# Agzs/BlockMaze

Measured on AMD Instinct MI355X. Metric: Groth16 proofs/sec (send circuit, alt_bn128), higher is better.
Workload: dtype u32 limbs (254-bit Fq/Fr Montgomery; all MSM accumulations, the H query's weighted bucket sum and the transforms' tiles on nine 29-bit limbs)

## Files before the change

### blockmaze_amd/csrc/capi_engine.cpp

```cpp
#include <cstring>
#include <memory>
#include <mutex>
#include <string>
#include <vector>
#include "../../include/zkgpu.h"
#include "gpu.hpp"
#include "capi_accounts.hpp"

namespace zk {
void probe_field(int field, int op, const uint8_t *a, const uint8_t *b, uint8_t *out, size_t n);
void probe_fq2(int op, const uint8_t *a, const uint8_t *b, uint8_t *out, size_t n);
void probe_group(int group, int op, const uint8_t *a, const uint8_t *b, uint8_t *out, size_t n);
void probe_field29(int field, int op, const uint32_t *a, const uint32_t *b, const uint32_t *c, const uint32_t *d, uint32_t *out, size_t n);
void probe_point29(int op, const uint32_t *a, const uint32_t *b, uint32_t *out, uint32_t *flags, size_t n);
void probe_fq2_sqrt(const uint8_t *a, uint8_t *out, uint8_t *ok, size_t n);
}
using namespace zk;
using namespace zk::host;

static thread_local std::string g_err;
void zkgpu_set_error(const std::string &s) { g_err = s; }
std::mutex g_gpu_mutex;

template <class Fn> static int guarded(Fn fn) {
// ... 153 lines not shown
void zkgpu_r1cs_destroy(zkgpu_r1cs *cs) { guarded([&] { delete cs; return ZKGPU_OK; }); }
int zkgpu_witness_map(zkgpu_r1cs *cs, const uint8_t *z, uint8_t *h_out) { return guarded([&] { if (!cs) return ZKGPU_ERR_ARG;
  size_t m = cs->dom->m(), nv = cs->host.n_vars; std::vector<Fe32> zz(nv + 1); memset(&zz[0], 0, 32); zz[0].l[0] = 1; if (nv) memcpy(&zz[1], z, 32 * nv);
  DevBuf<Fe32> zd(nv + 1), abc(3 * m); zd.upload(zz.data(), nv + 1); fr_to_mont_dev(zd.get(), nv + 1);
  cs->dev->eval(zd.get(), abc.get(), m);
  if (!cs->dev->satisfied(abc.get(), m)) {
    g_err = "assignment does not satisfy the constraint system";
    return ZKGPU_ERR_UNSATISFIED;
  }
  cs->dom->ifft(abc.get(), 3, m);
  cs->dom->coset_fft(abc.get(), 3, m);
  cs->dom->qap_pointwise(abc.get(), abc.get() + m, abc.get() + 2 * m);
  cs->dom->icoset_fft(abc.get(), 1, m);
  fr_from_mont_dev(abc.get(), m); abc.download((Fe32 *)h_out, m); memset(h_out + 32 * m, 0, 32); return ZKGPU_OK; }); }

int zkgpu_test_decompress(int group, const uint8_t *xs_mont, const uint8_t *flags, size_t n, uint8_t *points_out) {
  return guarded([&] { if (group != 1 && group != 2) { g_err = "group must be 1 or 2"; return ZKGPU_ERR_ARG; }
    if (group == 1) { std::vector<G1AffineRaw> p(n ? n : 1); decompress_g1((const Fe32 *)xs_mont, flags, n, p.data()); for (size_t i = 0; i < n; i++) g1_raw_out(p[i], points_out + 64 * i); }
    else { std::vector<G2AffineRaw> p(n ? n : 1); decompress_g2((const Fe32 *)xs_mont, flags, n, p.data()); for (size_t i = 0; i < n; i++) g2_raw_out(p[i], points_out + 128 * i); }
    return ZKGPU_OK; });
}
int zkgpu_test_fixed_base_mul(int group, const uint8_t *base, const uint8_t *scalars, size_t n, uint8_t *points_out) {
  return guarded([&] { if (group != 1 && group != 2) { g_err = "group must be 1 or 2"; return ZKGPU_ERR_ARG; }
    if (group == 1) { G1AffineRaw b; g1_to_raw(base, b); HFq x, y; memcpy(x.l, &b.x, 32); memcpy(y.l, &b.y, 32);
      std::vector<G1AffineRaw> p(n ? n : 1); fixed_base_mul_g1(HG1::from_affine(x, y), (const Fe32 *)scalars, n, p.data()); for (size_t i = 0; i < n; i++) g1_raw_out(p[i], points_out + 64 * i); }
    else { G2AffineRaw b; g2_to_raw(base, b); HFq2 x, y; memcpy(x.c0.l, &b.x0, 32); memcpy(x.c1.l, &b.x1, 32); memcpy(y.c0.l, &b.y0, 32); memcpy(y.c1.l, &b.y1, 32);
      std::vector<G2AffineRaw> p(n ? n : 1); fixed_base_mul_g2(HG2::from_affine(x, y), (const Fe32 *)scalars, n, p.data()); for (size_t i = 0; i < n; i++) g2_raw_out(p[i], points_out + 128 * i); }
    return ZKGPU_OK; });
}
int zkgpu_test_h_query_lagrange(size_t min_size, const uint8_t *h, size_t n_in, uint8_t *out) {
// ... 72 lines not shown
```

### blockmaze_amd/csrc/gpu.hip

```cpp
#include <hip/hip_runtime.h>
#include <cstdio>
#include <cstdlib>
#include <chrono>
#include <cstring>
#include <map>
#include <vector>
#include <algorithm>
#include <mutex>
#include <atomic>
#include <mutex>
#include "gpu_internal.hpp"
#include "ntt.cuh"
#include "ecntt.cuh"

__attribute__((constructor(101))) static void zkgpu_load_time_environment() { setenv("GPU_MAX_HW_QUEUES", "16", 0); }

namespace zk {

constexpr int MAX_LANES_PER_DEVICE = 31, MAX_LANES = 1 + 8 * 28;
static uint8_t g_lane_claimed[MAX_LANES];
static std::atomic<GpuContext *> g_lanes[MAX_LANES];
static std::atomic<int> g_lane_slot[MAX_LANES];
static std::mutex g_lane_mutex;
static thread_local int t_lane = 0;
// ... 198 lines not shown
    o.n_ = 0;
  }
  return *this;
}
template <class T> void DevBuf<T>::upload(const T *h, size_t n) {
  HIP_CHECK(hipMemcpyAsync(p_, h, n * sizeof(T), hipMemcpyHostToDevice, gpu().stream));
  HIP_CHECK(hipStreamSynchronize(gpu().stream));
}
template <class T> void DevBuf<T>::download(T *h, size_t n) const {
  HIP_CHECK(hipMemcpyAsync(h, p_, n * sizeof(T), hipMemcpyDeviceToHost, gpu().stream));
  HIP_CHECK(hipStreamSynchronize(gpu().stream));
}
template <class T> void DevBuf<T>::zero() { if (n_) HIP_CHECK(hipMemsetAsync(p_, 0, n_ * sizeof(T), gpu().stream)); }
template class DevBuf<uint8_t>;
template class DevBuf<uint32_t>;
template class DevBuf<Fe32>;
template class DevBuf<G1AffineRaw>;
template class DevBuf<G2AffineRaw>;

template <class T> PinnedBuf<T>::PinnedBuf(size_t n) : n_(n) { gpu(); if (n) { HIP_CHECK(hipHostMalloc((void **)&p_, n * sizeof(T))); if (alloc_poison()) memset(p_, 0xA5, n * sizeof(T)); } }
template <class T> PinnedBuf<T>::~PinnedBuf() { release(); }
template <class T> void PinnedBuf<T>::release() { if (p_) hipHostFree(p_); p_ = nullptr; n_ = 0; }
template class PinnedBuf<Fe32>;
void upload_async(void *dev, const void *host, size_t bytes) { HIP_CHECK(hipMemcpyAsync(dev, host, bytes, hipMemcpyHostToDevice, gpu().stream)); }
static __global__ void k_copy_words16(const uint4 *__restrict__ src, uint4 *__restrict__ dst, size_t n16) {
  for (size_t i = (size_t)blockIdx.x * blockDim.x + threadIdx.x; i < n16; i += (size_t)gridDim.x * blockDim.x) dst[i] = src[i];
}
void copy_dev_async(void *dst, const void *src, size_t bytes) {
  if (!bytes) return;
  if (bytes % 16 || (reinterpret_cast<uintptr_t>(dst) | reinterpret_cast<uintptr_t>(src)) % 16) { HIP_CHECK(hipMemcpyAsync(dst, src, bytes, hipMemcpyDeviceToDevice, gpu().stream)); return; }
// ... 479 lines not shown
  return d;
}
void gpu_host_unregister(void *p) { if (p) { (void)hipHostUnregister(p); (void)hipGetLastError(); } }
static std::atomic<uint64_t> g_general_path_repeats{0}, g_queries_without_tables{0};
uint64_t queries_without_tables() { return g_queries_without_tables.load(std::memory_order_relaxed); }
void note_query_without_tables() { g_queries_without_tables.fetch_add(1, std::memory_order_relaxed); }
uint64_t general_path_repeats() { return g_general_path_repeats.load(std::memory_order_relaxed); }
void note_general_path_repeat() { g_general_path_repeats.fetch_add(1, std::memory_order_relaxed); }
void merge_equal_columns_dev(Fe32 *z, uint8_t *tags, const uint32_t *grp_ptr, const uint32_t *grp_mem, size_t n_groups) {
  if (n_groups) hipLaunchKernelGGL(k_merge_equal_columns, dim3(cdiv(n_groups, 64)), dim3(64), 0, gpu().stream, (Fr *)z, tags, grp_ptr, grp_mem, (uint32_t)n_groups);
}
void fr_to_mont_dev(Fe32 *a, size_t n) { if (n) hipLaunchKernelGGL(k_fr_to_mont, dim3(cdiv(n, 256)), dim3(256), 0, gpu().stream, (Fr *)a, (uint32_t)n); }
void fr_from_mont_dev(Fe32 *a, size_t n) { if (n) hipLaunchKernelGGL(k_fr_from_mont, dim3(cdiv(n, 256)), dim3(256), 0, gpu().stream, (Fr *)a, (uint32_t)n); }

struct R1csArrays { size_t n_inputs, n_vars, n_cons; DevBuf<uint32_t> rowptr[3], col[3], cid[3], long_rows[3]; size_t n_long[3] = {0, 0, 0}; DevBuf<Fe32> ctab;
    DevBuf<uint32_t> long_any; size_t n_long_any = 0; };
struct R1csDev::Impl {
  std::shared_ptr<R1csArrays> a;
  size_t &n_inputs, &n_vars, &n_cons;
  DevBuf<uint32_t> (&rowptr)[3], (&col)[3], (&cid)[3], (&long_rows)[3];
  size_t (&n_long)[3];
  DevBuf<Fe32> &ctab;
  DevBuf<uint32_t> &long_any;
  size_t &n_long_any;
  DevBuf<uint32_t> flag;
  uint32_t *h_flag = nullptr;
  uint32_t *h_fail = nullptr, *d_fail = nullptr, seq = 0;
  explicit Impl(std::shared_ptr<R1csArrays> aa) : a(aa), n_inputs(a->n_inputs), n_vars(a->n_vars), n_cons(a->n_cons), rowptr(a->rowptr), col(a->col),
      cid(a->cid), long_rows(a->long_rows), n_long(a->n_long), ctab(a->ctab), long_any(a->long_any), n_long_any(a->n_long_any) {
  }
  void own_words() {
    flag = DevBuf<uint32_t>(1);
    HIP_CHECK(hipHostMalloc((void **)&h_flag, 4));
    HIP_CHECK(hipHostMalloc((void **)&h_fail, 8, hipHostMallocMapped));
    h_fail[0] = 0; h_fail[1] = 0;
    HIP_CHECK(hipHostGetDevicePointer((void **)&d_fail, h_fail, 0));
  }
  ~Impl() { if (h_flag) hipHostFree(h_flag); if (h_fail) hipHostFree(h_fail); }
};
R1csDev::R1csDev(const R1csDev &peer) : impl(new Impl(peer.impl->a)) { impl->own_words(); }
R1csDev::R1csDev(const R1csHost &h) : impl(new Impl(std::make_shared<R1csArrays>())) {
  Impl &d = *impl; d.n_inputs = h.n_inputs; d.n_vars = h.n_vars; d.n_cons = h.n_cons;
  std::vector<Fe32> tab(2); { HFr one = HFr::one(), m1 = one.neg(); memcpy(&tab[0], one.l, 32); memcpy(&tab[1], m1.l, 32); }
  struct Key { uint32_t l[8]; bool operator<(const Key &o) const { return memcmp(l, o.l, 32) < 0; } };
  std::vector<std::pair<Key, uint32_t>> seen;
  size_t cap = 1 << 12; std::vector<int64_t> slots(cap, -1); std::vector<Fe32> keys; std::vector<uint32_t> vals;
  auto lookup = [&](const Fe32 &c) -> uint32_t {
    uint64_t hsh = ((uint64_t)c.l[1] << 32 | c.l[0]) * 0x9E3779B97F4A7C15ull ^ c.l[7]; size_t pos = hsh & (cap - 1);
    for (;;) { int64_t s = slots[pos]; if (s < 0) break; if (!memcmp(&keys[s], &c, 32)) return vals[s]; pos = (pos + 1) & (cap - 1); }
    if (keys.size() * 2 >= cap) throw GpuError("r1cs: more than 2048 distinct coefficients");
    HFr v; memcpy(v.l, &c, 32); v = v.to_mont(); Fe32 m; memcpy(&m, v.l, 32); uint32_t id;
    if (!memcmp(&m, &tab[0], 32)) id = 0; else if (!memcmp(&m, &tab[1], 32)) id = 1; else { id = (uint32_t)tab.size(); tab.push_back(m); }
    slots[pos] = (int64_t)keys.size(); keys.push_back(c); vals.push_back(id); return id; };
  for (int m = 0; m < 3; m++) {
    if (h.rowptr[m].size() != h.n_cons + 1) throw GpuError("r1cs: rowptr size");
    std::vector<uint32_t> ids(h.col[m].size()); for (size_t k = 0; k < ids.size(); k++) ids[k] = lookup(h.coeff[m][k]);
    d.rowptr[m] = DevBuf<uint32_t>(h.n_cons + 1); d.rowptr[m].upload(h.rowptr[m].data(), h.n_cons + 1);
    d.col[m] = DevBuf<uint32_t>(ids.size() + 1); d.cid[m] = DevBuf<uint32_t>(ids.size() + 1);
    if (!ids.empty()) { d.col[m].upload(h.col[m].data(), ids.size()); d.cid[m].upload(ids.data(), ids.size()); }
    std::vector<uint32_t> lr; for (size_t i = 0; i < h.n_cons; i++) if (h.rowptr[m][i + 1] - h.rowptr[m][i] > R1CS_LONG_ROW) lr.push_back((uint32_t)i);
    d.n_long[m] = lr.size(); d.long_rows[m] = DevBuf<uint32_t>(lr.size() + 1); if (!lr.empty()) d.long_rows[m].upload(lr.data(), lr.size());
  }
  {
    std::vector<uint32_t> lr;
    for (size_t i = 0; i < h.n_cons; i++) {
      bool lg = false;
      for (int m = 0; m < 3; m++) lg |= h.rowptr[m][i + 1] - h.rowptr[m][i] > R1CS_LONG_ROW;
      if (lg) lr.push_back((uint32_t)i);
    }
    d.n_long_any = lr.size(); d.long_any = DevBuf<uint32_t>(lr.size() + 1); if (!lr.empty()) d.long_any.upload(lr.data(), lr.size()); }
  d.ctab = DevBuf<Fe32>(tab.size()); d.ctab.upload(tab.data(), tab.size()); d.own_words();
}
R1csDev::~R1csDev() = default;
void R1csDev::eval(const Fe32 *z, Fe32 *abc, size_t m, const uint8_t *tags, bool write_c) {
  Stage st("r1cs.rows"); Impl &d = *impl; hipStream_t s = gpu().stream; if (m < d.n_cons + d.n_inputs + 1) throw GpuError("r1cs: domain too small");
  R1csMatrices M; for (int mm = 0; mm < 3; mm++) { M.rowptr[mm] = d.rowptr[mm].get(); M.col[mm] = d.col[mm].get(); M.cid[mm] = d.cid[mm].get(); }
  if (++d.seq == 0) d.seq = 1;
  if (tags) {
    const uint32_t sb = (uint32_t)cdiv(m, 256);
    hipLaunchKernelGGL(k_r1cs_rows_tagged, dim3(sb + (unsigned)cdiv(d.n_long_any, 4)), dim3(256), 0, s, M, (const Fr *)d.ctab.get(), (const Fr *)z, tags,
        (uint32_t)d.n_cons, zk_with_prio(d.n_inputs, ZKP_ROWS), (uint32_t)m,
                       (const uint32_t *)d.long_any.get(), (uint32_t)d.n_long_any, sb, write_c ? 1 : 0, (Fr *)abc, d.seq, d.d_fail);
    return; }
  if (d.n_long_any) {
    const uint32_t sb = (uint32_t)cdiv(m, 256);
    hipLaunchKernelGGL(k_r1cs_rows_all, dim3(sb + (unsigned)cdiv(d.n_long_any, 4)), dim3(256), 0, s, M, (const Fr *)d.ctab.get(), (const Fr *)z,
        (uint32_t)d.n_cons, (uint32_t)d.n_inputs, (uint32_t)m, (const uint32_t *)d.long_any.get(), (uint32_t)d.n_long_any, sb, (Fr *)abc, d.seq, d.d_fail);
    return; }
  hipLaunchKernelGGL(k_r1cs_rows3, dim3(cdiv(m, 256)), dim3(256), 0, s, M, (const Fr *)d.ctab.get(), (const Fr *)z, (uint32_t)d.n_cons, (uint32_t)d.n_inputs,
      (uint32_t)m, (Fr *)abc, d.seq, d.d_fail);
  if (d.n_long_any) hipLaunchKernelGGL(k_r1cs_long_rows3, dim3((unsigned)d.n_long_any), dim3(64), 0, s, d.long_any.get(), M, (const Fr *)d.ctab.get(),
      (const Fr *)z, (uint32_t)m, (Fr *)abc, d.seq, d.d_fail);
}
bool R1csDev::check_result() const { return *impl->h_fail != impl->seq; }
uint32_t R1csDev::failed_row() const { return impl->h_fail[1]; }
bool R1csDev::satisfied(const Fe32 *abc, size_t m) {
  Impl &d = *impl; hipStream_t s = gpu().stream; d.flag.zero();
  if (d.n_cons) hipLaunchKernelGGL(k_r1cs_check, dim3(cdiv(d.n_cons, 256)), dim3(256), 0, s, (const Fr *)abc, (const Fr *)(abc + m), (const Fr *)(abc + 2 * m),
      (uint32_t)d.n_cons, d.flag.get());
  HIP_CHECK(hipMemcpyAsync(d.h_flag, d.flag.get(), 4, hipMemcpyDeviceToHost, s)); HIP_CHECK(hipStreamSynchronize(s)); return *d.h_flag == 0;
}

}
```

### blockmaze_amd/csrc/gpu.hpp

```cpp
#pragma once
#include <cstddef>
#include <cstdint>
#include <memory>
#include <stdexcept>
#include <string>
#include <vector>
#include "hostmath.hpp"
#include "pairing_host.hpp"

namespace zk {

struct GpuError : std::runtime_error { using std::runtime_error::runtime_error; };
struct GpuOutOfMemory : GpuError { using GpuError::GpuError; };
uint64_t queries_without_tables();
void note_query_without_tables();

struct Fe32 { uint32_t l[8]; };
struct G1AffineRaw { Fe32 x, y; };
struct G2AffineRaw { Fe32 x0, x1, y0, y1; };

class GpuContext;
GpuContext &gpu();
int gpu_device_numa_node(int device);
bool gpu_available();
// ... 195 lines not shown
  void coset_fft(Fe32 *data, int batch, size_t stride); void icoset_fft(Fe32 *data, int batch, size_t stride);
  void ifft_then_coset_fft(Fe32 *data, int batch, size_t stride);
 private: void fft_with_factors(Fe32 *data, int batch, size_t stride, const Fe32 *factors); public:
  bool supports_h_lagrange() const; void h_query_to_coset_lagrange(const G1AffineRaw *h, size_t n_in, G1AffineRaw *out );
  bool supports_c_fold() const;
  void fold_c_into_l(const G1AffineRaw *h_lagrange , const R1csHost &cs, const G1AffineRaw *L , G1AffineRaw *out);
  const Fe32 *zinv_dev() const; bool zinv_is_table() const;
  void qap_pointwise(Fe32 *a, const Fe32 *b, const Fe32 *c);
  struct Impl; std::unique_ptr<Impl> impl;
};

struct R1csHost {
  size_t n_inputs = 0, n_vars = 0, n_cons = 0;
  std::vector<uint32_t> rowptr[3], col[3]; std::vector<Fe32> coeff[3];
};
class R1csDev {
 public:
  explicit R1csDev(const R1csHost &h); explicit R1csDev(const R1csDev &peer); ~R1csDev();
  void eval(const Fe32 *z_dev, Fe32 *abc, size_t m, const uint8_t *tags_dev = nullptr, bool write_c = true);
  bool satisfied(const Fe32 *abc, size_t m);
  bool check_result() const;
  uint32_t failed_row() const;
  struct Impl; std::unique_ptr<Impl> impl;
};

void fr_to_mont_dev(Fe32 *a, size_t n); void fr_from_mont_dev(Fe32 *a, size_t n);
inline size_t expand_values_offset(size_t words, int canon) { return (((canon == 2 ? 28 : 20) * words + 31) / 32) * 32; }
void expand_witness_dev(const uint8_t *packed_dev, size_t words, const Fe32 &one_value, int canon, size_t n, Fe32 *out, uint8_t *tags_out = nullptr,
    uint32_t *other_vars_out = nullptr);
void expand_board_dev(const uint8_t *board_tags, size_t n, const uint32_t *cand, const Fe32 *cand_vals, size_t n_cand, Fe32 *z, uint8_t *tags, uint32_t *other_vars,
    uint32_t *counters, int parity, bool vals_by_var = false);
void merge_equal_columns_dev(Fe32 *z, uint8_t *tags, const uint32_t *grp_ptr, const uint32_t *grp_mem, size_t n_groups);
void classify_witness_dev(const Fe32 *z, size_t n, uint8_t *tags_out, uint32_t *other_vars_out, uint32_t *counters, int parity);

void decompress_g1(const Fe32 *xs, const uint8_t *flags, size_t n, G1AffineRaw *out);
void decompress_g2(const Fe32 *xs , const uint8_t *flags, size_t n, G2AffineRaw *out);
void fixed_base_mul_g1(const host::HG1 &base, const Fe32 *scalars, size_t n, G1AffineRaw *out);
// ... 18 lines not shown
```

### blockmaze_amd/csrc/ntt.cuh

```cuda
#pragma once
#include <hip/hip_runtime.h>
#include "field.cuh"
#include "field29.cuh"

namespace zk {

constexpr int NTT_LOCAL_LOG = 10;
constexpr int NTT_LOCAL_THREADS = 512;

__device__ __forceinline__ uint32_t bitrev32(uint32_t x, int bits) { return __brev(x) >> (32 - bits); }

__global__ void k_ntt_bitrev_scale(const Fr *__restrict__ in, Fr *__restrict__ out, const Fr *__restrict__ scale, int logn, size_t stride_in,
    size_t stride_out) {
  uint32_t i = blockIdx.x * blockDim.x + threadIdx.x, n = 1u << logn; if (i >= n) return;
  const Fr *src = in + blockIdx.y * stride_in; Fr *dst = out + blockIdx.y * stride_out; uint32_t r = bitrev32(i, logn);
  Fr v = src[r]; if (scale) v = v * scale[r]; dst[i] = v;
}

__global__ void __launch_bounds__(NTT_LOCAL_THREADS) k_ntt_local(Fr *__restrict__ data, const Fr *__restrict__ tw, int logn, int L, size_t stride) {
  extern __shared__ uint32_t lds_raw[]; Fr *tile = reinterpret_cast<Fr *>(lds_raw);
  const uint32_t T = 1u << L, half_n = 1u << (logn - 1); Fr *d = data + blockIdx.y * stride + (size_t)blockIdx.x * T;
  for (uint32_t i = threadIdx.x; i < T; i += blockDim.x) tile[i] = d[i];
  __syncthreads();
  for (int s = 1; s <= L; s++) {
// ... 379 lines not shown
    for (int d = 32; d >= 1; d >>= 1) {
      if ((uint32_t)d >= len) continue;
      Fr o;
      for (int i = 0; i < 8; i++) o.l[i] = __shfl_down(acc.l[i], d, 64);
      acc = acc + o;
    }
    v[mm] = acc;
  }
  if (lane == 0) {
    abc[r] = v[0];
    abc[m + r] = v[1];
    if (write_c) abc[2 * (size_t)m + r] = v[2];
    if (v[0] * v[1] != v[2]) { fail[1] = r; *fail = seq; }
  }
}
__global__ void k_r1cs_check(const Fr *__restrict__ a, const Fr *__restrict__ b, const Fr *__restrict__ c, uint32_t n_rows, uint32_t *flag) {
  uint32_t r = blockIdx.x * blockDim.x + threadIdx.x; if (r >= n_rows) return; if (a[r] * b[r] != c[r]) atomicOr(flag, 1u);
}

}
```

### blockmaze_amd/engine.py

```python
import ctypes, os
import numpy as np

_HERE = os.path.dirname(os.path.abspath(__file__))
LIB_PATH = os.path.join(_HERE, "libzkgpu.so")
if os.environ.get("ZKGPU_LIB"): LIB_PATH = os.environ["ZKGPU_LIB"]

class ZkGpuError(RuntimeError):
    pass

_lib = None
def lib():
    global _lib
    if _lib is None:
        if not os.path.exists(LIB_PATH):
            raise ZkGpuError("%s not built: run `python -c 'import __graft_entry__ as g; g.build()'` (hipcc, gfx950)" % LIB_PATH)
        L = ctypes.CDLL(LIB_PATH)
        L.zkgpu_last_error.restype = ctypes.c_char_p; L.zkgpu_version.restype = ctypes.c_char_p
        L.zkgpu_domain_size.restype = ctypes.c_size_t; L.zkgpu_domain_size.argtypes = [ctypes.c_size_t]
        L.zkgpu_msm_create.restype = ctypes.c_void_p; L.zkgpu_r1cs_create.restype = ctypes.c_void_p
        _lib = L
    return _lib

def _check(rc):
    if rc != 0:
# ... 166 lines not shown
class R1cs:
    def __init__(self, n_inputs, n_vars, n_cons, rowptr, col, coeff):
        self.n_inputs, self.n_vars, self.n_cons = n_inputs, n_vars, n_cons
        self._keep = [[np.ascontiguousarray(x, dtype=np.uint32) for x in rowptr], [np.ascontiguousarray(x, dtype=np.uint32) for x in col], [np.ascontiguousarray(x, dtype=np.uint64) for x in coeff]]
        P32 = ctypes.POINTER(ctypes.c_uint32); P8 = ctypes.POINTER(ctypes.c_uint8)
        rp = (P32 * 3)(*[x.ctypes.data_as(P32) for x in self._keep[0]]); cl = (P32 * 3)(*[x.ctypes.data_as(P32) for x in self._keep[1]]); co = (P8 * 3)(*[x.ctypes.data_as(P8) for x in self._keep[2]])
        self.h = lib().zkgpu_r1cs_create(ctypes.c_size_t(n_inputs), ctypes.c_size_t(n_vars), ctypes.c_size_t(n_cons), rp, cl, co)
        if not self.h: raise ZkGpuError(lib().zkgpu_last_error().decode())
        self.m = domain_size(n_cons + n_inputs + 1)
    def witness_map(self, z):
        z = np.ascontiguousarray(z, dtype=np.uint64); H = np.zeros((self.m + 1, 4), dtype=np.uint64)
        _check(lib().zkgpu_witness_map(ctypes.c_void_p(self.h), _bytes(z), _bytes(H))); return H
    def fold_c(self, h_lagrange, L):
        P = np.ascontiguousarray(h_lagrange, dtype=np.uint64); L = np.ascontiguousarray(L, dtype=np.uint64); assert P.size == 8 * self.m and L.size == 8 * (self.n_vars - self.n_inputs)
        out = np.zeros((self.n_vars + 1, 8), dtype=np.uint64); _check(lib().zkgpu_test_fold_c(ctypes.c_void_p(self.h), _bytes(P), _bytes(L), _bytes(out))); return out
    def close(self):
        if self.h: lib().zkgpu_r1cs_destroy(ctypes.c_void_p(self.h)); self.h = None
    def __del__(self):
        try: self.close()
        except Exception: pass

def decompress(group, xs_mont, flags):
    w = 4 * group; xs = np.ascontiguousarray(xs_mont, dtype=np.uint64).reshape(-1, w); n = xs.shape[0]; f = np.ascontiguousarray(flags, dtype=np.uint8); assert f.shape == (n,)
    out = np.zeros((n, 8 * group), dtype=np.uint64); _check(lib().zkgpu_test_decompress(int(group), _bytes(xs), _bytes(f), ctypes.c_size_t(n), _bytes(out))); return out
def fixed_base_mul(group, base, scalars):
    b = np.ascontiguousarray(base, dtype=np.uint64).reshape(8 * group); k = np.ascontiguousarray(scalars, dtype=np.uint64).reshape(-1, 4); n = k.shape[0]
    out = np.zeros((n, 8 * group), dtype=np.uint64); _check(lib().zkgpu_test_fixed_base_mul(int(group), _bytes(b), _bytes(k), ctypes.c_size_t(n), _bytes(out))); return out
def h_query_lagrange(min_size, h):
    h = np.ascontiguousarray(h, dtype=np.uint64).reshape(-1, 8); out = np.zeros((domain_size(min_size), 8), dtype=np.uint64)
    _check(lib().zkgpu_test_h_query_lagrange(ctypes.c_size_t(min_size), _bytes(h), ctypes.c_size_t(h.shape[0]), _bytes(out))); return out

KIND = {"mint": 0, "send": 1, "deposit": 2, "redeem": 3, "sha256": 100, "merkle": 101, "lesscmp": 102, "cmta": 103, "cmts": 104, "prf": 105, "crh": 106, "unpacker": 107}
def circuit_export(kind, path, tree_depth=8): _check(lib().zkgpu_circuit_export(KIND[kind], tree_depth, path.encode()))
def keygen(kind, pk_path, vk_path, seed=0, tree_depth=8): _check(lib().zkgpu_keygen(KIND[kind], tree_depth, ctypes.c_uint64(seed), pk_path.encode(), vk_path.encode()))
def keygen_from_r1cs(r1cs_path, pk_path, vk_path, seed=0): _check(lib().zkgpu_keygen_from_r1cs(r1cs_path.encode(), ctypes.c_uint64(seed), pk_path.encode(), vk_path.encode()))
# ... 604 lines not shown
```

### include/zkgpu.h

```cpp
#ifndef ZKGPU_H
#define ZKGPU_H
#include <stddef.h>
#include <stdint.h>
#include "zk_records.h"
#ifdef __cplusplus
extern "C" {
#endif

#define ZKGPU_OK 0
#define ZKGPU_ERR_NO_DEVICE (-1)
#define ZKGPU_ERR_ARG (-2)
#define ZKGPU_ERR_RUNTIME (-3)
#define ZKGPU_ERR_UNSATISFIED (-4)

const char *zkgpu_last_error(void);
const char *zkgpu_version(void);
int zkgpu_device_count(void);
int zkgpu_device_numa_node(int device);
int zkgpu_init(void);

int zkgpu_test_field_op(int field, int op, const uint8_t *a, const uint8_t *b, uint8_t *out, size_t n);
int zkgpu_test_fq2_op(int op, const uint8_t *a, const uint8_t *b, uint8_t *out, size_t n);
int zkgpu_test_group_op(int group, int op, const uint8_t *a, const uint8_t *b, uint8_t *out, size_t n);
int zkgpu_test_field29_op(int field, int op, const uint32_t *a, const uint32_t *b, const uint32_t *c, const uint32_t *d, uint32_t *out, size_t n);
// ... 12 lines not shown
int zkgpu_test_msm_run_product(zkgpu_msm *h, const uint8_t *a, const uint8_t *b, const uint8_t *z, int z_is_table, uint8_t out[64]);
int zkgpu_test_msm_h_state(zkgpu_msm *h, int what, uint32_t *out, size_t cap_words, size_t *words);

size_t zkgpu_domain_size(size_t min_size);
int zkgpu_domain_transform(size_t min_size, int op, uint8_t *data);

typedef struct zkgpu_r1cs zkgpu_r1cs;
zkgpu_r1cs *zkgpu_r1cs_create(size_t n_inputs, size_t n_vars, size_t n_cons, const uint32_t *const rowptr[3], const uint32_t *const col[3], const uint8_t *const coeff[3]);
void zkgpu_r1cs_destroy(zkgpu_r1cs *cs);
int zkgpu_witness_map(zkgpu_r1cs *cs, const uint8_t *z, uint8_t *h_out);

int zkgpu_test_decompress(int group, const uint8_t *xs_mont, const uint8_t *flags, size_t n, uint8_t *points_out);
int zkgpu_test_fixed_base_mul(int group, const uint8_t *base, const uint8_t *scalars, size_t n, uint8_t *points_out);
int zkgpu_test_h_query_lagrange(size_t min_size, const uint8_t *h, size_t n_in, uint8_t *out);
int zkgpu_test_fold_c(zkgpu_r1cs *cs, const uint8_t *h_lagrange, const uint8_t *L, uint8_t *out);

int zkgpu_circuit_export(int kind, int tree_depth, const char *r1cs_path);
int zkgpu_witness_sha256(const uint8_t left[32], const uint8_t right[32], const char *wit_path);
int zkgpu_witness_lesscmp(uint64_t value_old, uint64_t value_s, const char *wit_path);
int zkgpu_witness_unpacker(int nbits, const uint8_t *bits , const char *wit_path);
int zkgpu_witness_hashblock(int which , const uint8_t *bits , const char *wit_path);
int zkgpu_witness_cmta(const uint8_t *bits , const char *wit_path);
int zkgpu_witness_send(uint64_t value_A, char *r_s, char *sn, char *r, char *cmt_s, char *cmtA, uint64_t value_s, char *pk_recv, uint64_t value_A_new, char *sn_A_new,
                       char *r_A_new, char *cmt_A_new, char *sk, char *pk_sender, const char *wit_path);
int zkgpu_witness_deposit(uint64_t value, uint64_t value_old, char *sn_old, char *r_old, char *sn, char *r, char *sns, char *rs, char *cmtB_old, char *cmtB, uint64_t value_s, char *pk,
                          char *sn_A_old, char *cmtS, char *cmtarray, int n, char *sk, int tree_depth, const char *wit_path);
int zkgpu_witness_merkle(int depth, const uint8_t leaf[32], const uint8_t *siblings, uint64_t position, const char *wit_path);
int zkgpu_witness_mint_redeem(int redeem, uint64_t value, uint64_t value_old, char *sn_old, char *r_old, char *sn, char *r, char *cmtA_old, char *cmtA, uint64_t value_s, char *sk, const char *wit_path);
int zkgpu_keygen(int kind, int tree_depth, uint64_t seed, const char *pk_path, const char *vk_path);
int zkgpu_keygen_from_r1cs(const char *r1cs_path, uint64_t seed, const char *pk_path, const char *vk_path);
// ... 149 lines not shown
```

Before: 1287.

## Add packed R1CS row kernel with integer coefficient sums for one-valued witnesses

Packs the three constraint matrices into one interleaved term stream per row, with 21-bit column and coefficient-id fields and per-row length words. Long rows get separate records handled by groups of lanes. Terms whose witness value is tagged one and whose coefficient is a small integer are summed as 64-bit integers and converted to a field element once per row, which avoids per-term Montgomery field additions and multiplications. The path becomes the default whenever witness tags are supplied and the system fits the packed limits. The cost is extra host packing at setup, more device buffers, and added branch divergence in the kernel.

```diff
diff --git a/blockmaze_amd/csrc/capi_engine.cpp b/blockmaze_amd/csrc/capi_engine.cpp
--- a/blockmaze_amd/csrc/capi_engine.cpp
+++ b/blockmaze_amd/csrc/capi_engine.cpp
@@ -191,6 +191,43 @@
   cs->dom->icoset_fft(abc.get(), 1, m);
   fr_from_mont_dev(abc.get(), m); abc.download((Fe32 *)h_out, m); memset(h_out + 32 * m, 0, 32); return ZKGPU_OK; }); }
 
+static void r1cs_host_from(R1csHost &h, size_t n_inputs, size_t n_vars, size_t n_cons, const uint32_t *const rowptr[3], const uint32_t *const col[3],
+    const uint8_t *const coeff[3]) {
+  h.n_inputs = n_inputs; h.n_vars = n_vars; h.n_cons = n_cons;
+  for (int m = 0; m < 3; m++) {
+    const size_t nnz = rowptr[m][n_cons];
+    h.rowptr[m].assign(rowptr[m], rowptr[m] + n_cons + 1); h.col[m].assign(col[m], col[m] + nnz); h.coeff[m].resize(nnz);
+    if (nnz) memcpy(h.coeff[m].data(), coeff[m], 32 * nnz);
+  }
+}
+int zkgpu_test_r1cs_pack(size_t n_inputs, size_t n_vars, size_t n_cons, const uint32_t *const rowptr[3], const uint32_t *const col[3], const uint8_t *const coeff[3],
+    uint32_t *terms, uint32_t *rows, uint32_t *long_recs, int64_t *classes, uint8_t *ctab, size_t counts[4]) {
+  try {
+    if (!rowptr || !col || !coeff || !counts) { g_err = "r1cs pack: arguments"; return ZKGPU_ERR_ARG; }
+    R1csHost h; r1cs_host_from(h, n_inputs, n_vars, n_cons, rowptr, col, coeff); R1csPacked p; r1cs_pack(h, p);
+    counts[0] = p.ok ? 1 : 0; counts[1] = p.terms.size(); counts[2] = p.long_recs.size() / 4; counts[3] = p.cls.size();
+    if (terms && !p.terms.empty()) memcpy(terms, p.terms.data(), 4 * p.terms.size());
+    if (rows && !p.rows.empty()) memcpy(rows, p.rows.data(), 4 * p.rows.size());
+    if (long_recs && !p.long_recs.empty()) memcpy(long_recs, p.long_recs.data(), 4 * p.long_recs.size());
+    if (classes) memcpy(classes, p.cls.data(), 8 * p.cls.size());
+    if (ctab) memcpy(ctab, p.ctab.data(), 32 * p.ctab.size());
+    return ZKGPU_OK;
+  }
+  catch (const std::exception &e) { g_err = e.what(); return ZKGPU_ERR_RUNTIME; }
+  catch (...) { g_err = "unknown error"; return ZKGPU_ERR_RUNTIME; }
+}
+int zkgpu_test_r1cs_rows(zkgpu_r1cs *cs, const uint8_t *z, int mode, int write_c, uint8_t *abc, uint32_t fail_out[2]) { return guarded([&] {
+  if (!cs || !z || !abc || !fail_out || mode < 0) { g_err = "r1cs rows: arguments"; return ZKGPU_ERR_ARG; }
+  const size_t m = cs->dom->m(), nv = cs->host.n_vars, n = nv + 1; std::vector<Fe32> zz(n); memset(&zz[0], 0, 32); zz[0].l[0] = 1; if (nv) memcpy(&zz[1], z, 32 * nv);
+  DevBuf<Fe32> zd(n), out(3 * m); DevBuf<uint8_t> tags(n); DevBuf<uint32_t> others(n), counters(2);
+  zd.upload(zz.data(), n); fr_to_mont_dev(zd.get(), n); out.upload((const Fe32 *)abc, 3 * m); counters.zero();
+  classify_witness_dev(zd.get(), n, tags.get(), others.get(), counters.get(), 0);
+  if (mode & (1 << 17)) { gpu_sync(); const std::vector<uint8_t> all(n, 2); tags.upload(all.data(), n); }
+  cs->dev->eval(zd.get(), out.get(), m, tags.get(), write_c != 0, mode & ~(1 << 17)); gpu_sync();
+  out.download((Fe32 *)abc, 3 * m); const bool ok = cs->dev->check_result(); cs->dev->fail_words(fail_out);
+  if (!ok) { g_err = "assignment does not satisfy the constraint system"; return ZKGPU_ERR_UNSATISFIED; }
+  return ZKGPU_OK; }); }
+
 int zkgpu_test_decompress(int group, const uint8_t *xs_mont, const uint8_t *flags, size_t n, uint8_t *points_out) {
   return guarded([&] { if (group != 1 && group != 2) { g_err = "group must be 1 or 2"; return ZKGPU_ERR_ARG; }
     if (group == 1) { std::vector<G1AffineRaw> p(n ? n : 1); decompress_g1((const Fe32 *)xs_mont, flags, n, p.data()); for (size_t i = 0; i < n; i++) g1_raw_out(p[i], points_out + 64 * i); }
diff --git a/blockmaze_amd/csrc/gpu.hip b/blockmaze_amd/csrc/gpu.hip
--- a/blockmaze_amd/csrc/gpu.hip
+++ b/blockmaze_amd/csrc/gpu.hip
@@ -236,6 +236,7 @@
 template <class T> void DevBuf<T>::zero() { if (n_) HIP_CHECK(hipMemsetAsync(p_, 0, n_ * sizeof(T), gpu().stream)); }
 template class DevBuf<uint8_t>;
 template class DevBuf<uint32_t>;
+template class DevBuf<int64_t>;
 template class DevBuf<Fe32>;
 template class DevBuf<G1AffineRaw>;
 template class DevBuf<G2AffineRaw>;
@@ -745,7 +746,8 @@
 void fr_from_mont_dev(Fe32 *a, size_t n) { if (n) hipLaunchKernelGGL(k_fr_from_mont, dim3(cdiv(n, 256)), dim3(256), 0, gpu().stream, (Fr *)a, (uint32_t)n); }
 
 struct R1csArrays { size_t n_inputs, n_vars, n_cons; DevBuf<uint32_t> rowptr[3], col[3], cid[3], long_rows[3]; size_t n_long[3] = {0, 0, 0}; DevBuf<Fe32> ctab;
-    DevBuf<uint32_t> long_any; size_t n_long_any = 0; };
+    DevBuf<uint32_t> long_any; size_t n_long_any = 0;
+    bool packed = false; DevBuf<uint32_t> p_rows, p_terms, p_long; DevBuf<int64_t> p_cls; size_t p_n_long = 0, p_n_coeff = 0; };
 struct R1csDev::Impl {
   std::shared_ptr<R1csArrays> a;
   size_t &n_inputs, &n_vars, &n_cons;
@@ -769,23 +771,52 @@
   }
   ~Impl() { if (h_flag) hipHostFree(h_flag); if (h_fail) hipHostFree(h_fail); }
 };
-R1csDev::R1csDev(const R1csDev &peer) : impl(new Impl(peer.impl->a)) { impl->own_words(); }
-R1csDev::R1csDev(const R1csHost &h) : impl(new Impl(std::make_shared<R1csArrays>())) {
-  Impl &d = *impl; d.n_inputs = h.n_inputs; d.n_vars = h.n_vars; d.n_cons = h.n_cons;
-  std::vector<Fe32> tab(2); { HFr one = HFr::one(), m1 = one.neg(); memcpy(&tab[0], one.l, 32); memcpy(&tab[1], m1.l, 32); }
-  struct Key { uint32_t l[8]; bool operator<(const Key &o) const { return memcmp(l, o.l, 32) < 0; } };
-  std::vector<std::pair<Key, uint32_t>> seen;
+void r1cs_pack(const R1csHost &h, R1csPacked &o) {
+  o = R1csPacked(); o.ctab.resize(2); { HFr one = HFr::one(), m1 = one.neg(); memcpy(&o.ctab[0], one.l, 32); memcpy(&o.ctab[1], m1.l, 32); }
+  const auto int_class = [](const Fe32 &c) -> int64_t {
+    const auto small = [](const uint32_t *l) { for (int i = 2; i < 8; i++) if (l[i]) return false; return l[1] < (1u << 8); };
+    if (small(c.l)) return (int64_t)((uint64_t)c.l[1] << 32 | c.l[0]);
+    uint32_t d[8]; uint64_t br = 0; for (int i = 0; i < 8; i++) { const uint64_t t = (uint64_t)FrParams::MOD[i] - c.l[i] - br; d[i] = (uint32_t)t; br = (t >> 32) & 1; }
+    if (!br && small(d)) return -(int64_t)((uint64_t)d[1] << 32 | d[0]);
+    return R1CS_NO_INT; };
+  o.cls.assign(2, 0); o.cls[0] = 1; o.cls[1] = -1;
   size_t cap = 1 << 12; std::vector<int64_t> slots(cap, -1); std::vector<Fe32> keys; std::vector<uint32_t> vals;
   auto lookup = [&](const Fe32 &c) -> uint32_t {
     uint64_t hsh = ((uint64_t)c.l[1] << 32 | c.l[0]) * 0x9E3779B97F4A7C15ull ^ c.l[7]; size_t pos = hsh & (cap - 1);
     for (;;) { int64_t s = slots[pos]; if (s < 0) break; if (!memcmp(&keys[s], &c, 32)) return vals[s]; pos = (pos + 1) & (cap - 1); }
     if (keys.size() * 2 >= cap) throw GpuError("r1cs: more than 2048 distinct coefficients");
     HFr v; memcpy(v.l, &c, 32); v = v.to_mont(); Fe32 m; memcpy(&m, v.l, 32); uint32_t id;
-    if (!memcmp(&m, &tab[0], 32)) id = 0; else if (!memcmp(&m, &tab[1], 32)) id = 1; else { id = (uint32_t)tab.size(); tab.push_back(m); }
+    if (!memcmp(&m, &o.ctab[0], 32)) id = 0; else if (!memcmp(&m, &o.ctab[1], 32)) id = 1; else { id = (uint32_t)o.ctab.size(); o.ctab.push_back(m); o.cls.push_back(int_class(c)); }
     slots[pos] = (int64_t)keys.size(); keys.push_back(c); vals.push_back(id); return id; };
+  size_t nnz = 0; bool fits = true;
   for (int m = 0; m < 3; m++) {
     if (h.rowptr[m].size() != h.n_cons + 1) throw GpuError("r1cs: rowptr size");
-    std::vector<uint32_t> ids(h.col[m].size()); for (size_t k = 0; k < ids.size(); k++) ids[k] = lookup(h.coeff[m][k]);
+    if (h.col[m].size() < h.rowptr[m][h.n_cons] || h.coeff[m].size() < h.col[m].size()) throw GpuError("r1cs: term arrays shorter than the row pointers say");
+    o.cid[m].resize(h.col[m].size()); for (size_t k = 0; k < o.cid[m].size(); k++) o.cid[m][k] = lookup(h.coeff[m][k]);
+    for (size_t k = 0; k < h.col[m].size(); k++) { if (h.col[m][k] > h.n_vars) throw GpuError("r1cs: a column beyond the variables"); fits &= h.col[m][k] <= R1CS_COL_MASK; }
+    for (size_t i = 0; i < h.n_cons; i++) { if (h.rowptr[m][i + 1] < h.rowptr[m][i]) throw GpuError("r1cs: row pointers decrease"); fits &= h.rowptr[m][i + 1] - h.rowptr[m][i] <= R1CS_LEN_MASK; }
+    nnz += h.rowptr[m][h.n_cons];
+  }
+  static_assert(((uint64_t)R1CS_LEN_MASK << 40) < ((uint64_t)1 << 62), "a row's integer sum must stay below 2^62");
+  if (!fits || nnz >= ((uint64_t)1 << 32)) return;
+  o.terms.reserve(nnz); o.rows.resize(2 * h.n_cons);
+  for (size_t i = 0; i < h.n_cons; i++) {
+    uint32_t lens = 0; bool lg = false; const uint32_t first = (uint32_t)o.terms.size();
+    for (int m = 0; m < 3; m++) {
+      const uint32_t lo = h.rowptr[m][i], hi = h.rowptr[m][i + 1]; lens |= (hi - lo) << (R1CS_LEN_BITS * m); lg |= hi - lo > R1CS_LONG_ROW;
+      for (uint32_t k = lo; k < hi; k++) o.terms.push_back(h.col[m][k] | o.cid[m][k] << R1CS_COL_BITS);
+    }
+    if (lg) { lens |= R1CS_REC_LONG; const uint32_t rec[4] = {(uint32_t)i, first, lens, 0}; o.long_recs.insert(o.long_recs.end(), rec, rec + 4); }
+    o.rows[2 * i] = first; o.rows[2 * i + 1] = lens;
+  }
+  o.ok = true;
+}
+R1csDev::R1csDev(const R1csDev &peer) : impl(new Impl(peer.impl->a)) { impl->own_words(); }
+R1csDev::R1csDev(const R1csHost &h) : impl(new Impl(std::make_shared<R1csArrays>())) {
+  Impl &d = *impl; d.n_inputs = h.n_inputs; d.n_vars = h.n_vars; d.n_cons = h.n_cons;
+  R1csPacked pk; r1cs_pack(h, pk);
+  for (int m = 0; m < 3; m++) {
+    const std::vector<uint32_t> &ids = pk.cid[m];
     d.rowptr[m] = DevBuf<uint32_t>(h.n_cons + 1); d.rowptr[m].upload(h.rowptr[m].data(), h.n_cons + 1);
     d.col[m] = DevBuf<uint32_t>(ids.size() + 1); d.cid[m] = DevBuf<uint32_t>(ids.size() + 1);
     if (!ids.empty()) { d.col[m].upload(h.col[m].data(), ids.size()); d.cid[m].upload(ids.data(), ids.size()); }
@@ -800,13 +831,37 @@
       if (lg) lr.push_back((uint32_t)i);
     }
     d.n_long_any = lr.size(); d.long_any = DevBuf<uint32_t>(lr.size() + 1); if (!lr.empty()) d.long_any.upload(lr.data(), lr.size()); }
-  d.ctab = DevBuf<Fe32>(tab.size()); d.ctab.upload(tab.data(), tab.size()); d.own_words();
+  d.ctab = DevBuf<Fe32>(pk.ctab.size()); d.ctab.upload(pk.ctab.data(), pk.ctab.size());
+  if (pk.ok) {
+    R1csArrays &a = *d.a; a.packed = true; a.p_n_long = pk.long_recs.size() / 4; a.p_n_coeff = pk.cls.size();
+    a.p_rows = DevBuf<uint32_t>(pk.rows.size() + 2); if (!pk.rows.empty()) a.p_rows.upload(pk.rows.data(), pk.rows.size());
+    a.p_terms = DevBuf<uint32_t>(pk.terms.size() + 1); if (!pk.terms.empty()) a.p_terms.upload(pk.terms.data(), pk.terms.size());
+    a.p_long = DevBuf<uint32_t>(pk.long_recs.size() + 4); if (!pk.long_recs.empty()) a.p_long.upload(pk.long_recs.data(), pk.long_recs.size());
+    a.p_cls = DevBuf<int64_t>(pk.cls.size()); a.p_cls.upload(pk.cls.data(), pk.cls.size());
+  }
+  d.own_words();
 }
 R1csDev::~R1csDev() = default;
-void R1csDev::eval(const Fe32 *z, Fe32 *abc, size_t m, const uint8_t *tags, bool write_c) {
+template <int G, bool CLS_LDS> static void launch_rows_packed(const R1csArrays &a, const R1csPackedDev &P, const Fe32 *ctab, const Fe32 *z, const uint8_t *tags, size_t m,
+    bool write_c, Fe32 *abc, uint32_t seq, uint32_t *d_fail) {
+  const uint32_t sb = (uint32_t)cdiv(m, 256), lb = (uint32_t)cdiv(a.p_n_long, 256 / G);
+  hipLaunchKernelGGL((k_r1cs_rows_packed<G, CLS_LDS>), dim3(lb + sb), dim3(256), CLS_LDS ? a.p_n_coeff * sizeof(int64_t) : 0, gpu().stream,
+      P, (const Fr *)ctab, (const Fr *)z, tags, (uint32_t)a.n_cons, zk_with_prio(a.n_inputs, ZKP_ROWS), (uint32_t)m, lb, write_c ? 1 : 0, (Fr *)abc, seq, d_fail);
+}
+bool R1csDev::packed() const { return impl->a->packed; }
+void R1csDev::eval(const Fe32 *z, Fe32 *abc, size_t m, const uint8_t *tags, bool write_c, int mode) {
   Stage st("r1cs.rows"); Impl &d = *impl; hipStream_t s = gpu().stream; if (m < d.n_cons + d.n_inputs + 1) throw GpuError("r1cs: domain too small");
   R1csMatrices M; for (int mm = 0; mm < 3; mm++) { M.rowptr[mm] = d.rowptr[mm].get(); M.col[mm] = d.col[mm].get(); M.cid[mm] = d.cid[mm].get(); }
   if (++d.seq == 0) d.seq = 1;
+  if (mode > 0 && !(tags && d.a->packed)) throw GpuError("r1cs: the packed row kernel needs tags and a system that was packed");
+  if (tags && d.a->packed && mode != 0) {
+    const R1csArrays &a = *d.a;
+    const R1csPackedDev P{(const uint2 *)a.p_rows.get(), a.p_terms.get(), (const uint4 *)a.p_long.get(), a.p_cls.get(), (uint32_t)a.p_n_long, (uint32_t)a.p_n_coeff};
+    const int g = mode > 0 && ((mode >> 8) & 0xff) ? (mode >> 8) & 0xff : R1CS_LONG_GROUP; const bool cls_global = mode > 0 && ((mode >> 16) & 1);
+#define ZK_ROWS_PACKED(G) (cls_global ? launch_rows_packed<G, false> : launch_rows_packed<G, true>)(a, P, d.ctab.get(), z, tags, m, write_c, abc, d.seq, d.d_fail)
+    if (g == 8) ZK_ROWS_PACKED(8); else if (g == 16) ZK_ROWS_PACKED(16); else if (g == 32) ZK_ROWS_PACKED(32); else throw GpuError("r1cs: a long row's group has 8, 16 or 32 lanes");
+#undef ZK_ROWS_PACKED
+    return; }
   if (tags) {
     const uint32_t sb = (uint32_t)cdiv(m, 256);
     hipLaunchKernelGGL(k_r1cs_rows_tagged, dim3(sb + (unsigned)cdiv(d.n_long_any, 4)), dim3(256), 0, s, M, (const Fr *)d.ctab.get(), (const Fr *)z, tags,
@@ -823,6 +878,7 @@
   if (d.n_long_any) hipLaunchKernelGGL(k_r1cs_long_rows3, dim3((unsigned)d.n_long_any), dim3(64), 0, s, d.long_any.get(), M, (const Fr *)d.ctab.get(),
       (const Fr *)z, (uint32_t)m, (Fr *)abc, d.seq, d.d_fail);
 }
+void R1csDev::fail_words(uint32_t out[2]) const { out[0] = impl->h_fail[0]; out[1] = impl->h_fail[1]; }
 bool R1csDev::check_result() const { return *impl->h_fail != impl->seq; }
 uint32_t R1csDev::failed_row() const { return impl->h_fail[1]; }
 bool R1csDev::satisfied(const Fe32 *abc, size_t m) {
diff --git a/blockmaze_amd/csrc/gpu.hpp b/blockmaze_amd/csrc/gpu.hpp
--- a/blockmaze_amd/csrc/gpu.hpp
+++ b/blockmaze_amd/csrc/gpu.hpp
@@ -233,13 +233,17 @@
   size_t n_inputs = 0, n_vars = 0, n_cons = 0;
   std::vector<uint32_t> rowptr[3], col[3]; std::vector<Fe32> coeff[3];
 };
+struct R1csPacked { bool ok = false; std::vector<uint32_t> terms, rows, long_recs, cid[3]; std::vector<int64_t> cls; std::vector<Fe32> ctab; };
+void r1cs_pack(const R1csHost &h, R1csPacked &out);
 class R1csDev {
  public:
   explicit R1csDev(const R1csHost &h); explicit R1csDev(const R1csDev &peer); ~R1csDev();
-  void eval(const Fe32 *z_dev, Fe32 *abc, size_t m, const uint8_t *tags_dev = nullptr, bool write_c = true);
+  void eval(const Fe32 *z_dev, Fe32 *abc, size_t m, const uint8_t *tags_dev = nullptr, bool write_c = true, int mode = -1);
+  bool packed() const;
   bool satisfied(const Fe32 *abc, size_t m);
   bool check_result() const;
   uint32_t failed_row() const;
+  void fail_words(uint32_t out[2]) const;
   struct Impl; std::unique_ptr<Impl> impl;
 };
 
diff --git a/blockmaze_amd/csrc/ntt.cuh b/blockmaze_amd/csrc/ntt.cuh
--- a/blockmaze_amd/csrc/ntt.cuh
+++ b/blockmaze_amd/csrc/ntt.cuh
@@ -417,6 +417,139 @@
     if (v[0] * v[1] != v[2]) { fail[1] = r; *fail = seq; }
   }
 }
+constexpr uint32_t R1CS_COL_BITS = 21, R1CS_COL_MASK = (1u << R1CS_COL_BITS) - 1;
+constexpr uint32_t R1CS_LEN_BITS = 10, R1CS_LEN_MASK = (1u << R1CS_LEN_BITS) - 1, R1CS_REC_LONG = 1u << 30;
+constexpr int64_t R1CS_NO_INT = INT64_MIN;
+constexpr int R1CS_PREFETCH = 16;
+constexpr int R1CS_LONG_BATCH = 4;
+constexpr int R1CS_LONG_GROUP = 16;
+struct R1csPackedDev { const uint2 *rows; const uint32_t *terms; const uint4 *long_recs; const int64_t *cls; uint32_t n_long, n_coeff; };
+
+template <int N> __device__ __forceinline__ uint32_t r1cs_pick(const uint32_t (&t)[N], uint32_t j) {
+  uint32_t v = 0;
+#pragma unroll
+  for (int k = 0; k < N; k++) v |= t[k] & (0u - (uint32_t)(j == (uint32_t)k));
+  return v;
+}
+__device__ __forceinline__ void r1cs_field_term(Fr (&f)[3], uint32_t mm, uint32_t term, bool coef_only, const Fr *__restrict__ ctab, const Fr *__restrict__ z) {
+  const uint32_t col = term & R1CS_COL_MASK, ci = term >> R1CS_COL_BITS;
+  Fr x = coef_only ? ctab[ci] : z[col];
+  if (__ballot(!coef_only && ci > 1)) { const Fr p = ctab[ci] * x; if (!coef_only && ci > 1) x = p; }
+  if (!coef_only && ci == 1) x = x.neg();
+  const uint32_t m0 = mm == 0 ? ~0u : 0u, m1 = mm == 1 ? ~0u : 0u, m2 = mm == 2 ? ~0u : 0u; Fr t;
+#pragma unroll
+  for (int i = 0; i < 8; i++) t.l[i] = (f[0].l[i] & m0) | (f[1].l[i] & m1) | (f[2].l[i] & m2);
+  t = t + x;
+#pragma unroll
+  for (int i = 0; i < 8; i++) { f[0].l[i] = (f[0].l[i] & ~m0) | (t.l[i] & m0); f[1].l[i] = (f[1].l[i] & ~m1) | (t.l[i] & m1); f[2].l[i] = (f[2].l[i] & ~m2) | (t.l[i] & m2); }
+}
+__device__ __forceinline__ Fr r1cs_row_value(int64_t s, const Fr &f, bool has_field) {
+  const bool neg = s < 0; const uint64_t mag = neg ? (uint64_t)0 - (uint64_t)s : (uint64_t)s;
+  Fr v = Fr::zero();
+  if (__ballot(mag > 3)) { v.l[0] = (uint32_t)mag; v.l[1] = (uint32_t)(mag >> 32); v = v.to_mont(); }
+  else {
+    const Fr one = Fr::one(); if (mag & 1) v = one;
+    if (__ballot(mag & 2)) { const Fr two = one + one; v = v + ((mag & 2) ? two : Fr::zero()); }
+  }
+  if (__ballot(neg)) { if (neg) v = v.neg(); }
+  if (__ballot(has_field)) v = v + f;
+  return v;
+}
+__device__ __forceinline__ bool r1cs_row_violated(const Fr &a, const Fr &b, const Fr &c) {
+  const Fr one = Fr::one(); bool bad = false, general = false;
+  if (a.is_zero() || b.is_zero()) bad = !c.is_zero();
+  else if (a == one) bad = b != c;
+  else if (b == one) bad = a != c;
+  else general = true;
+  if (__ballot(general)) { const Fr p = a * b; if (general) bad = p != c; }
+  return bad;
+}
+template <int G, bool CLS_LDS>
+__global__ void __launch_bounds__(256) k_r1cs_rows_packed(R1csPackedDev P, const Fr *__restrict__ ctab, const Fr *__restrict__ z, const uint8_t *__restrict__ tags,
+    uint32_t n_rows, uint32_t n_inputs, uint32_t m, uint32_t long_blocks, int write_c, Fr *__restrict__ abc, uint32_t seq, uint32_t *fail) {
+  zk_take_prio(n_inputs);
+  extern __shared__ int64_t s_cls[];
+  const bool short_rows = blockIdx.x >= long_blocks; uint32_t r = 0; bool have = false; uint2 rec = make_uint2(0, 0); uint4 lrec = make_uint4(0, 0, 0, 0);
+  if (short_rows) { r = (blockIdx.x - long_blocks) * 256u + threadIdx.x; if (r < n_rows) rec = P.rows[r]; }
+  else { const uint32_t w = blockIdx.x * (256u / G) + threadIdx.x / G; have = w < P.n_long; if (have) lrec = P.long_recs[w]; }
+  if (CLS_LDS) { for (uint32_t i = threadIdx.x; i < P.n_coeff; i += 256) s_cls[i] = P.cls[i]; __syncthreads(); }
+  const int64_t *__restrict__ cls = CLS_LDS ? s_cls : P.cls;
+  int64_t s[3] = {0, 0, 0}; Fr f[3] = {Fr::zero(), Fr::zero(), Fr::zero()}; uint32_t fused = 0; bool live;
+  if (short_rows) {
+    if (r >= m) return;
+    if (r >= n_rows) {
+      abc[r] = r <= n_rows + n_inputs ? z[r - n_rows] : Fr::zero();
+      abc[m + r] = Fr::zero();
+      if (write_c) abc[2 * (size_t)m + r] = Fr::zero();
+      return;
+    }
+    live = !(rec.y & R1CS_REC_LONG);
+    const uint32_t nA = rec.y & R1CS_LEN_MASK, nAB = nA + ((rec.y >> R1CS_LEN_BITS) & R1CS_LEN_MASK), total = live ? nAB + ((rec.y >> 2 * R1CS_LEN_BITS) & R1CS_LEN_MASK) : 0u;
+    for (uint32_t base = 0; __ballot(base < total); base += R1CS_PREFETCH) {
+      uint32_t t[R1CS_PREFETCH]; uint8_t tg[R1CS_PREFETCH];
+#pragma unroll
+      for (int j = 0; j < R1CS_PREFETCH; j++) t[j] = base + j < total ? P.terms[rec.x + base + j] : 0u;
+#pragma unroll
+      for (int j = 0; j < R1CS_PREFETCH; j++) tg[j] = base + j < total ? tags[t[j] & R1CS_COL_MASK] : ZTAG_ZERO;
+      uint32_t f_other = 0, f_coef = 0;
+#pragma unroll
+      for (int j = 0; j < R1CS_PREFETCH; j++) {
+        const uint32_t pos = base + j;
+        if (!__ballot(pos < total)) break;
+        if (tg[j] == ZTAG_ZERO) continue;
+        if (tg[j] != ZTAG_ONE) { f_other |= 1u << j; continue; }
+        const int64_t c = cls[t[j] >> R1CS_COL_BITS];
+        if (c == R1CS_NO_INT) f_coef |= 1u << j; else if (pos < nA) s[0] += c; else if (pos < nAB) s[1] += c; else s[2] += c;
+      }
+      for (uint32_t fm = f_other | f_coef; fm; fm &= fm - 1) {
+        const uint32_t j = (uint32_t)__builtin_ctz(fm), pos = base + j, mm = (pos >= nA) + (pos >= nAB);
+        r1cs_field_term(f, mm, r1cs_pick(t, j), (f_coef >> j) & 1, ctab, z); fused |= 1u << mm;
+      }
+    }
+  } else {
+    const uint32_t gl = threadIdx.x % G; const uint4 rec = lrec;
+    r = rec.x; live = have && gl == 0;
+    const uint32_t nA = rec.z & R1CS_LEN_MASK, nAB = nA + ((rec.z >> R1CS_LEN_BITS) & R1CS_LEN_MASK), total = nAB + ((rec.z >> 2 * R1CS_LEN_BITS) & R1CS_LEN_MASK);
+    for (uint32_t base = gl; __ballot(base < total); base += G * R1CS_LONG_BATCH) {
+      uint32_t t[R1CS_LONG_BATCH]; uint8_t tg[R1CS_LONG_BATCH];
+#pragma unroll
+      for (int j = 0; j < R1CS_LONG_BATCH; j++) t[j] = base + j * G < total ? P.terms[rec.y + base + j * G] : 0u;
+#pragma unroll
+      for (int j = 0; j < R1CS_LONG_BATCH; j++) tg[j] = base + j * G < total ? tags[t[j] & R1CS_COL_MASK] : ZTAG_ZERO;
+      uint32_t f_other = 0, f_coef = 0;
+#pragma unroll
+      for (int j = 0; j < R1CS_LONG_BATCH; j++) {
+        const uint32_t pos = base + j * G;
+        if (tg[j] == ZTAG_ZERO) continue;
+        if (tg[j] != ZTAG_ONE) { f_other |= 1u << j; continue; }
+        const int64_t c = cls[t[j] >> R1CS_COL_BITS];
+        if (c == R1CS_NO_INT) f_coef |= 1u << j; else if (pos < nA) s[0] += c; else if (pos < nAB) s[1] += c; else s[2] += c;
+      }
+      for (uint32_t fm = f_other | f_coef; fm; fm &= fm - 1) {
+        const uint32_t j = (uint32_t)__builtin_ctz(fm), pos = base + j * G, mm = (pos >= nA) + (pos >= nAB);
+        r1cs_field_term(f, mm, r1cs_pick(t, j), (f_coef >> j) & 1, ctab, z); fused |= 1u << mm;
+      }
+    }
+#pragma unroll
+    for (int mm = 0; mm < 3; mm++) {
+#pragma unroll
+      for (int d = G / 2; d >= 1; d >>= 1) s[mm] += __shfl_down(s[mm], d, G);
+      if (__ballot((fused >> mm) & 1)) {
+#pragma unroll 1
+        for (int d = G / 2; d >= 1; d >>= 1) { Fr o; for (int i = 0; i < 8; i++) o.l[i] = __shfl_down(f[mm].l[i], d, G); f[mm] = f[mm] + o; }
+        fused |= 1u << mm;
+      }
+    }
+    if (!live) { s[0] = s[1] = s[2] = 0; f[0] = f[1] = f[2] = Fr::zero(); }
+  }
+  const Fr a = r1cs_row_value(s[0], f[0], fused & 1), b = r1cs_row_value(s[1], f[1], (fused >> 1) & 1), c = r1cs_row_value(s[2], f[2], (fused >> 2) & 1);
+  const bool bad = r1cs_row_violated(a, b, c);
+  if (!live) return;
+  abc[r] = a;
+  abc[m + r] = b;
+  if (write_c) abc[2 * (size_t)m + r] = c;
+  if (bad) { fail[1] = r; *fail = seq; }
+}
 __global__ void k_r1cs_check(const Fr *__restrict__ a, const Fr *__restrict__ b, const Fr *__restrict__ c, uint32_t n_rows, uint32_t *flag) {
   uint32_t r = blockIdx.x * blockDim.x + threadIdx.x; if (r >= n_rows) return; if (a[r] * b[r] != c[r]) atomicOr(flag, 1u);
 }
diff --git a/blockmaze_amd/engine.py b/blockmaze_amd/engine.py
--- a/blockmaze_amd/engine.py
+++ b/blockmaze_amd/engine.py
@@ -204,11 +204,29 @@
     def fold_c(self, h_lagrange, L):
         P = np.ascontiguousarray(h_lagrange, dtype=np.uint64); L = np.ascontiguousarray(L, dtype=np.uint64); assert P.size == 8 * self.m and L.size == 8 * (self.n_vars - self.n_inputs)
         out = np.zeros((self.n_vars + 1, 8), dtype=np.uint64); _check(lib().zkgpu_test_fold_c(ctypes.c_void_p(self.h), _bytes(P), _bytes(L), _bytes(out))); return out
+    def rows(self, z, mode=1, write_c=True, abc=None, lanes=0, classes_global=False, all_other=False):
+        z = np.ascontiguousarray(z, dtype=np.uint64); assert z.size == 4 * self.n_vars
+        out = np.zeros((3, self.m, 4), dtype=np.uint64) if abc is None else np.ascontiguousarray(abc, dtype=np.uint64).reshape(3, self.m, 4).copy()
+        fail = np.zeros(2, dtype=np.uint32); full = int(mode) | (int(lanes) << 8 if mode else 0) | ((1 << 16) if classes_global and mode else 0) | ((1 << 17) if all_other else 0)
+        rc = lib().zkgpu_test_r1cs_rows(ctypes.c_void_p(self.h), _bytes(z), full, int(bool(write_c)), _bytes(out), _u32(fail))
+        if rc not in (0, -4): _check(rc)
+        return out, fail, rc == -4
     def close(self):
         if self.h: lib().zkgpu_r1cs_destroy(ctypes.c_void_p(self.h)); self.h = None
     def __del__(self):
         try: self.close()
         except Exception: pass
+
+def r1cs_pack(n_inputs, n_vars, n_cons, rowptr, col, coeff):
+    keep = [[np.ascontiguousarray(x, dtype=np.uint32) for x in rowptr], [np.ascontiguousarray(x, dtype=np.uint32) for x in col], [np.ascontiguousarray(x, dtype=np.uint64) for x in coeff]]
+    P32 = ctypes.POINTER(ctypes.c_uint32); P8 = ctypes.POINTER(ctypes.c_uint8)
+    rp = (P32 * 3)(*[x.ctypes.data_as(P32) for x in keep[0]]); cl = (P32 * 3)(*[x.ctypes.data_as(P32) for x in keep[1]]); co = (P8 * 3)(*[x.ctypes.data_as(P8) for x in keep[2]])
+    nnz = sum(int(x[n_cons]) for x in keep[0]); terms = np.zeros(max(1, nnz), dtype=np.uint32); rows = np.zeros((max(1, n_cons), 2), dtype=np.uint32)
+    longs = np.zeros((max(1, n_cons), 4), dtype=np.uint32); cls = np.zeros(2048, dtype=np.int64); ctab = np.zeros((2048, 4), dtype=np.uint64); counts = (ctypes.c_size_t * 4)()
+    _check(lib().zkgpu_test_r1cs_pack(ctypes.c_size_t(n_inputs), ctypes.c_size_t(n_vars), ctypes.c_size_t(n_cons), rp, cl, co, _u32(terms), _u32(rows), _u32(longs),
+                                      cls.ctypes.data_as(ctypes.POINTER(ctypes.c_int64)), _bytes(ctab), counts))
+    ok, nt, nl, nc = (int(c) for c in counts)
+    return dict(packed=bool(ok), terms=terms[:nt], rows=rows[:n_cons] if ok else rows[:0], long_recs=longs[:nl], classes=cls[:nc], ctab=ctab[:nc])
 
 def decompress(group, xs_mont, flags):
     w = 4 * group; xs = np.ascontiguousarray(xs_mont, dtype=np.uint64).reshape(-1, w); n = xs.shape[0]; f = np.ascontiguousarray(flags, dtype=np.uint8); assert f.shape == (n,)
diff --git a/include/zkgpu.h b/include/zkgpu.h
--- a/include/zkgpu.h
+++ b/include/zkgpu.h
@@ -50,6 +50,9 @@
 int zkgpu_test_fixed_base_mul(int group, const uint8_t *base, const uint8_t *scalars, size_t n, uint8_t *points_out);
 int zkgpu_test_h_query_lagrange(size_t min_size, const uint8_t *h, size_t n_in, uint8_t *out);
 int zkgpu_test_fold_c(zkgpu_r1cs *cs, const uint8_t *h_lagrange, const uint8_t *L, uint8_t *out);
+int zkgpu_test_r1cs_pack(size_t n_inputs, size_t n_vars, size_t n_cons, const uint32_t *const rowptr[3], const uint32_t *const col[3], const uint8_t *const coeff[3],
+    uint32_t *terms, uint32_t *rows, uint32_t *long_recs, int64_t *classes, uint8_t *ctab, size_t counts[4]);
+int zkgpu_test_r1cs_rows(zkgpu_r1cs *cs, const uint8_t *z, int mode, int write_c, uint8_t *abc, uint32_t fail_out[2]);
 
 int zkgpu_circuit_export(int kind, int tree_depth, const char *r1cs_path);
 int zkgpu_witness_sha256(const uint8_t left[32], const uint8_t right[32], const char *wit_path);
```

Result: slower. 1269 (-1.4%).
